# zhaoshan2/pangu-pytorch

Hardware: AMD Instinct MI355X
Metric: forward steps/sec (721x1440x13pl) per MI355X (higher is better)
Workload: dtype f32; 1 GPU; PanguModel fp32 forward, 1 sample/GPU, input (1,5,13,721,1440)+(1,4,721,1440), depths 2-6-6-2, dims 192/384, random-init weights (BASELINE configs[1]); parallelism=dp1

## Files before the change

pangu-pytorch_amd/csrc/gemm_f32_split.hip:

```cpp
#include "split_f32.h"

namespace {

using namespace pangu_split;

using Tile = SplitTile<2, 2, 3>;
constexpr int BM = Tile::BM;
constexpr int BN = Tile::BN;

__global__ __launch_bounds__(256) void split_weight_kernel(const float* __restrict__ W, unsigned char* __restrict__ image, int N,
                                                           int K) {
  const int kc = K >> 3;
  const long long t = (long long)blockIdx.x * 256 + threadIdx.x;
  if (t >= (long long)N * kc) return;
  const int n = (int)(t / kc), c = (int)(t - (long long)n * kc);
  const float* src = W + (size_t)n * K + c * 8;
  const f32x4 c0 = *reinterpret_cast<const f32x4*>(src), c1 = *reinterpret_cast<const f32x4*>(src + 4);
  bf16x8 p[3];
  split8(c0, c1, p[0], p[1], p[2]);
  const int nt = n / BN, nl = n - nt * BN, kt = c >> 1, lh = c & 1;
  unsigned char* dst = image + ((size_t)nt * (K / BK) + kt) * B_BYTES + (lh * BN + nl) * 16;
#pragma unroll
  for (int q = 0; q < 3; ++q) *reinterpret_cast<bf16x8*>(dst + q * PLANE) = p[q];
}

template <int ACT, bool HAS_BIAS>
__global__ __launch_bounds__(256, 2) void gemm_f32_split_kernel(const float* __restrict__ A, int lda,
                                                                const unsigned char* __restrict__ image,
                                                                const float* __restrict__ bias, float* __restrict__ C, int ldc,
                                                                int M, int N, int K, int m_tiles, int n_tiles) {
  __shared__ __attribute__((aligned(16))) unsigned char smem[Tile::SMEM];

  const int b = blockIdx.x;
  const int xcd = b & 7, local = b >> 3;
  const int m_tile = (local / n_tiles) * 8 + xcd;
  const int n_tile = local % n_tiles;
  if (m_tile >= m_tiles) return;
  const int m0 = m_tile * BM, n0 = n_tile * BN;

  const int lane = threadIdx.x & 63;
  const int wave = __builtin_amdgcn_readfirstlane(threadIdx.x >> 6);
  const int wm = wave >> 1, wn = wave & 1;
  const int lr = lane & 31, lh = lane >> 5;

  f32x16 acc[2][3];
  split_main_loop<2, 2, 3>(smem, A, lda, image, M, N, K, m0, n_tile, acc);

  constexpr int EP_LD = 36;
  float* ep = reinterpret_cast<float*>(smem) + wave * (32 * EP_LD);
  const int er = lane >> 3, ec = (lane & 7) * 4;
  const __amdgpu_buffer_rsrc_t c_rsrc = __builtin_amdgcn_make_buffer_rsrc(
      C, 0, (int)(((size_t)(M - 1) * ldc + N) * sizeof(float)), 0x00020000);
#pragma unroll
  for (int j = 0; j < 3; ++j) {
    const int col = n0 + wn * 96 + j * 32 + ec;
    f32x4 bv = {0.f, 0.f, 0.f, 0.f};
    if (HAS_BIAS) bv = *reinterpret_cast<const f32x4*>(bias + col);
#pragma unroll
    for (int i = 0; i < 2; ++i) {
#pragma unroll
      for (int r = 0; r < 16; ++r) ep[((r & 3) + 8 * (r >> 2) + 4 * lh) * EP_LD + lr] = acc[i][j][r];
      const int row0 = m0 + wm * 64 + i * 32 + er;
#pragma unroll
      for (int it = 0; it < 4; ++it) {
        f32x4 v = *reinterpret_cast<const f32x4*>(&ep[(er + 8 * it) * EP_LD + ec]);
        v += bv;
        if (ACT == PANGU_ACT_GELU) {
#pragma unroll
          for (int c = 0; c < 4; ++c) v[c] = gelu_erf(v[c]);
        }
        const unsigned off = ((unsigned)(row0 + 8 * it) * (unsigned)ldc + (unsigned)col) * 4u;
        __builtin_amdgcn_raw_buffer_store_b128(__builtin_bit_cast(u32x4, v), c_rsrc, (int)off, 0, 2);
      }
    }
  }
}

}

extern "C" int pangu_split_weight_bf16x3(pangu_stream_t stream, const float* W, int N, int K, void* image) {
  if (!W || !image) return PANGU_E_NULL;
  if (N <= 0 || K <= 0 || (N % BN) != 0 || (K % BK) != 0) return PANGU_E_SHAPE;
  if ((long long)N * K * 6 >= 0xFFFFFFFFll) return PANGU_E_RANGE;
  const long long threads = (long long)N * (K / 8);
  hipLaunchKernelGGL(split_weight_kernel, dim3((unsigned)((threads + 255) / 256)), dim3(256), 0, (hipStream_t)stream, W,
                     reinterpret_cast<unsigned char*>(image), N, K);
  return pangu_launch_status();
}

extern "C" int pangu_linear_fwd_split(pangu_stream_t stream, const float* A, int lda, const void* image, const float* bias,
                                      float* C, int ldc, int M, int N, int K, int act) {
  if (!A || !image || !C) return PANGU_E_NULL;
  if (M <= 0 || N <= 0 || K <= 0 || lda < K || ldc < N || (lda & 3) || (ldc & 3)) return PANGU_E_SHAPE;
  if (act != PANGU_ACT_NONE && act != PANGU_ACT_GELU) return PANGU_E_ARG;
  if ((N % BN) != 0 || (K % BK) != 0) return PANGU_E_SHAPE;
  if (!pangu_fits_u32(M, lda, 4) || !pangu_fits_u32(M, ldc, 4) || (long long)N * K * 6 >= 0xFFFFFFFFll) return PANGU_E_RANGE;
  const int m_tiles = (M + BM - 1) / BM, n_tiles = N / BN;
  const dim3 g(((m_tiles + 7) / 8) * 8 * n_tiles), blk(256);
  hipStream_t s = (hipStream_t)stream;
  const unsigned char* img = reinterpret_cast<const unsigned char*>(image);
#define PANGU_SPLIT_LAUNCH(ACT, HB) \
  hipLaunchKernelGGL((gemm_f32_split_kernel<ACT, HB>), g, blk, 0, s, A, lda, img, bias, C, ldc, M, N, K, m_tiles, n_tiles)
  if (act == PANGU_ACT_GELU) {
    if (bias) PANGU_SPLIT_LAUNCH(PANGU_ACT_GELU, true); else PANGU_SPLIT_LAUNCH(PANGU_ACT_GELU, false);
  } else {
    if (bias) PANGU_SPLIT_LAUNCH(PANGU_ACT_NONE, true); else PANGU_SPLIT_LAUNCH(PANGU_ACT_NONE, false);
  }
#undef PANGU_SPLIT_LAUNCH
  return pangu_launch_status();
}
```

pangu-pytorch_amd/csrc/gemm_ln_f32_split.hip:

```cpp
#include "ln_epilogue_f32.h"
#include "split_f32.h"

namespace {

using namespace pangu_split;

template <int WMW, int WNW, int NST, bool HAS_BIAS>
__global__ __launch_bounds__(64 * WMW * WNW, WMW * WNW == 8 ? 1 : 2) void gemm_ln_residual_f32_split_kernel(
    const float* __restrict__ A, int lda, const unsigned char* __restrict__ image, const float* __restrict__ bias,
    const float* __restrict__ shortcut, int lds_sc, const float* __restrict__ gamma, const float* __restrict__ beta,
    float* __restrict__ C, int ldc, int M, int K, float branch_scale) {
  using Tile = SplitTile<WMW, WNW, NST>;
  __shared__ __attribute__((aligned(16))) unsigned char smem[Tile::SMEM];
  const int m0 = blockIdx.x * Tile::BM;
  f32x16 acc[2][3];
  split_main_loop<WMW, WNW, NST>(smem, A, lda, image, M, Tile::BN, K, m0, 0, acc);
  pangu_ln::ln_residual_epilogue<WMW, WNW, HAS_BIAS, false>(smem, acc, bias, shortcut, lds_sc, gamma, beta, C, ldc, M, m0,
                                                           branch_scale);
}

template <int WMW, int WNW, int NST>
int launch_ln_split(hipStream_t s, const float* A, int lda, const unsigned char* image, const float* bias, const float* shortcut,
                    int lds, const float* gamma, const float* beta, float* out, int ldo, int M, int K, float branch_scale) {
  constexpr int BM = 64 * WMW;
  dim3 g((M + BM - 1) / BM), blk(64 * WMW * WNW);
  if (bias)
    hipLaunchKernelGGL((gemm_ln_residual_f32_split_kernel<WMW, WNW, NST, true>), g, blk, 0, s, A, lda, image, bias, shortcut, lds,
                       gamma, beta, out, ldo, M, K, branch_scale);
  else
    hipLaunchKernelGGL((gemm_ln_residual_f32_split_kernel<WMW, WNW, NST, false>), g, blk, 0, s, A, lda, image, bias, shortcut, lds,
                       gamma, beta, out, ldo, M, K, branch_scale);
  return pangu_launch_status();
}

}

extern "C" int pangu_linear_ln_residual_fwd_split(pangu_stream_t stream, const float* A, int lda, const void* image,
                                                  const float* bias, const float* shortcut, int lds, const float* gamma,
                                                  const float* beta, float* out, int ldo, int M, int N, int K,
                                                  float branch_scale) {
  if (!A || !image || !shortcut || !gamma || !beta || !out) return PANGU_E_NULL;
  if (M <= 0 || K <= 0 || (K % BK) != 0 || lda < K || (lda & 3) || ldo < N || (ldo & 3) || lds < N || (lds & 3))
    return PANGU_E_SHAPE;
  if (N != 192 && N != 384) return PANGU_E_SHAPE;
  if (!pangu_fits_u32(M, lda, 4) || !pangu_fits_u32(M, ldo, 4) || !pangu_fits_u32(M, lds, 4) ||
      (long long)N * K * 6 >= 0xFFFFFFFFll)
    return PANGU_E_RANGE;
  hipStream_t s = (hipStream_t)stream;
  const unsigned char* img = reinterpret_cast<const unsigned char*>(image);
  if (N == 192) return launch_ln_split<2, 2, 3>(s, A, lda, img, bias, shortcut, lds, gamma, beta, out, ldo, M, K, branch_scale);
  return launch_ln_split<1, 4, 2>(s, A, lda, img, bias, shortcut, lds, gamma, beta, out, ldo, M, K, branch_scale);
}
```

pangu-pytorch_amd/csrc/ln_epilogue_f32.h:

```cpp
#pragma once
#include "common.h"

namespace pangu_ln {

constexpr float LN_EPS = 1e-5f;

__device__ inline float oct_sum(float v) {
  v += __builtin_bit_cast(float, __builtin_amdgcn_update_dpp(0, __builtin_bit_cast(int, v), 0xB1, 0xF, 0xF, true));
  v += __builtin_bit_cast(float, __builtin_amdgcn_update_dpp(0, __builtin_bit_cast(int, v), 0x4E, 0xF, 0xF, true));
  v += __builtin_bit_cast(float, __builtin_amdgcn_update_dpp(0, __builtin_bit_cast(int, v), 0x141, 0xF, 0xF, true));
  return v;
}

template <int WMW, int WNW, bool HAS_BIAS, bool PIN_COL>
__device__ __forceinline__ void ln_residual_epilogue(unsigned char* smem, const f32x16 (&acc)[2][3], const float* __restrict__ bias,
                                                     const float* __restrict__ shortcut, int lds_sc,
                                                     const float* __restrict__ gamma, const float* __restrict__ beta,
                                                     float* __restrict__ C, int ldc, int M, int m0, float branch_scale) {
  constexpr int NW = WMW * WNW;
  constexpr int BN = 96 * WNW;
  constexpr int EP_LD = 36;
  constexpr float INV_C = 1.0f / BN;
  const int lane = threadIdx.x & 63;
  const int wave = __builtin_amdgcn_readfirstlane(threadIdx.x >> 6);
  const int wm = wave / WNW, wn = wave % WNW;
  const int lr = lane & 31, lh = lane >> 5;
  float* ep = reinterpret_cast<float*>(smem) + wave * (32 * EP_LD);
  float* stats = reinterpret_cast<float*>(smem) + NW * (32 * EP_LD);
  const int er = lane >> 3, ec = (lane & 7) * 4;
  const __amdgpu_buffer_rsrc_t c_rsrc = __builtin_amdgcn_make_buffer_rsrc(
      C, 0, (int)(((size_t)(M - 1) * ldc + BN) * sizeof(float)), 0x00020000);
  const __amdgpu_buffer_rsrc_t s_rsrc = __builtin_amdgcn_make_buffer_rsrc(
      const_cast<float*>(shortcut), 0, (int)(((size_t)(M - 1) * lds_sc + BN) * sizeof(float)), 0x00020000);
#pragma unroll
  for (int i = 0; i < 2; ++i) {
    f32x4 y[3][4];
    float s[4] = {0.f, 0.f, 0.f, 0.f}, q[4] = {0.f, 0.f, 0.f, 0.f};
#pragma unroll
    for (int j = 0; j < 3; ++j) {
      int col = wn * 96 + j * 32 + ec;
      if (PIN_COL) asm volatile("" : "+v"(col));
      f32x4 bv = {0.f, 0.f, 0.f, 0.f};
      if (HAS_BIAS) bv = *reinterpret_cast<const f32x4*>(bias + col);
#pragma unroll
      for (int r = 0; r < 16; ++r) ep[((r & 3) + 8 * (r >> 2) + 4 * lh) * EP_LD + lr] = acc[i][j][r];
#pragma unroll
      for (int it = 0; it < 4; ++it) {
        f32x4 v = *reinterpret_cast<const f32x4*>(&ep[(er + 8 * it) * EP_LD + ec]);
        v += bv;
        y[j][it] = v;
        s[it] += (v[0] + v[1]) + (v[2] + v[3]);
        q[it] += (v[0] * v[0] + v[1] * v[1]) + (v[2] * v[2] + v[3] * v[3]);
      }
    }
#pragma unroll
    for (int it = 0; it < 4; ++it) {
      const float ss = oct_sum(s[it]), qq = oct_sum(q[it]);
      if ((lane & 7) == 0) {
        float* st = stats + (((wm * WNW + wn) * 64) + i * 32 + er + 8 * it) * 2;
        st[0] = ss;
        st[1] = qq;
      }
    }
    __syncthreads();
    float mean[4], rstd[4];
#pragma unroll
    for (int it = 0; it < 4; ++it) {
      const int rloc = i * 32 + er + 8 * it;
      float ts = 0.f, tq = 0.f;
#pragma unroll
      for (int w = 0; w < WNW; ++w) {
        const float* st = stats + ((wm * WNW + w) * 64 + rloc) * 2;
        ts += st[0];
        tq += st[1];
      }
      mean[it] = ts * INV_C;
      rstd[it] = rsqrtf(fmaxf(tq * INV_C - mean[it] * mean[it], 0.f) + LN_EPS);
    }
#pragma unroll
    for (int j = 0; j < 3; ++j) {
      int col = wn * 96 + j * 32 + ec;
      if (PIN_COL) asm volatile("" : "+v"(col));
      const f32x4 gm = *reinterpret_cast<const f32x4*>(gamma + col);
      const f32x4 bt = *reinterpret_cast<const f32x4*>(beta + col);
#pragma unroll
      for (int it = 0; it < 4; ++it) {
        const unsigned row = (unsigned)(m0 + wm * 64 + i * 32 + er + 8 * it);
        const f32x4 sc = __builtin_bit_cast(
            f32x4, __builtin_amdgcn_raw_buffer_load_b128(s_rsrc, (int)((row * (unsigned)lds_sc + (unsigned)col) * 4u), 0, 0));
        const f32x4 v = sc + branch_scale * ((y[j][it] - mean[it]) * rstd[it] * gm + bt);
        __builtin_amdgcn_raw_buffer_store_b128(__builtin_bit_cast(u32x4, v), c_rsrc,
                                               (int)((row * (unsigned)ldc + (unsigned)col) * 4u), 0, 0);
      }
    }
  }
}

}
```

pangu-pytorch_amd/csrc/split_f32.h:

```cpp
#pragma once
#include "gemm_f32_dma_loop.h"

namespace pangu_split {

using pangu_dma::BK;
using pangu_dma::kswz64;

typedef short bf16x8 __attribute__((ext_vector_type(8)));

constexpr int W_ROWS = 192;
constexpr int PLANE = 2 * W_ROWS * 16;
constexpr int B_BYTES = 3 * PLANE;
constexpr int W_PIECES = B_BYTES / 1024;

__device__ inline void split2(float a, float b, unsigned& hi, unsigned& mid, unsigned& lo) {
  const bf16x2_t h = __builtin_convertvector(f32x2_t{a, b}, bf16x2_t);
  const f32x2_t r1 = f32x2_t{a, b} - __builtin_convertvector(h, f32x2_t);
  const bf16x2_t m = __builtin_convertvector(r1, bf16x2_t);
  const f32x2_t r2 = r1 - __builtin_convertvector(m, f32x2_t);
  hi = __builtin_bit_cast(unsigned, h);
  mid = __builtin_bit_cast(unsigned, m);
  lo = __builtin_bit_cast(unsigned, __builtin_convertvector(r2, bf16x2_t));
}

__device__ inline void split8(const f32x4 c0, const f32x4 c1, bf16x8& hi, bf16x8& mid, bf16x8& lo) {
  unsigned h0, h1, h2, h3, m0, m1, m2, m3, l0, l1, l2, l3;
  split2(c0[0], c0[1], h0, m0, l0);
  split2(c0[2], c0[3], h1, m1, l1);
  split2(c1[0], c1[1], h2, m2, l2);
  split2(c1[2], c1[3], h3, m3, l3);
  hi = __builtin_bit_cast(bf16x8, u32x4{h0, h1, h2, h3});
  mid = __builtin_bit_cast(bf16x8, u32x4{m0, m1, m2, m3});
  lo = __builtin_bit_cast(bf16x8, u32x4{l0, l1, l2, l3});
}

template <int WMW, int WNW, int NST>
struct SplitTile {
  static constexpr int NW = WMW * WNW;
  static constexpr int BM = 64 * WMW;
  static constexpr int BN = 96 * WNW;
  static constexpr int NT = BN / W_ROWS;
  static constexpr int A_BYTES = BM * 64;
  static constexpr int STAGE = A_BYTES + NT * B_BYTES;
  static constexpr int SMEM = NST * STAGE;
  static_assert(NST == 2 || NST == 3, "ring depth");
  static_assert(BN % W_ROWS == 0, "whole n-tile blocks");
};

template <int WMW, int WNW, int NST>
__device__ __forceinline__ void split_main_loop(unsigned char* smem, const float* __restrict__ A, int lda,
                                                const unsigned char* __restrict__ image, int M, int N, int K, int m0,
                                                int first_n_tile, f32x16 (&acc)[2][3]) {
  using T = SplitTile<WMW, WNW, NST>;
  constexpr int NW = T::NW, A_BYTES = T::A_BYTES, STAGE = T::STAGE;
  constexpr int A_PIECES = A_BYTES / 1024;
  constexpr int PIECES = STAGE / 1024;
  constexpr int A_IT = A_PIECES / NW;
  constexpr int IT = (PIECES + NW - 1) / NW;
  constexpr int REM = PIECES % NW;
  static_assert(A_PIECES % NW == 0, "piece rounds");

  const int tid = threadIdx.x, lane = tid & 63;
  const int wave = __builtin_amdgcn_readfirstlane(tid >> 6);
  const int wm = wave / WNW, wn = wave % WNW;
  const int lr = lane & 31, lh = lane >> 5;
  const int KT = K / BK;

  const __amdgpu_buffer_rsrc_t a_rsrc = __builtin_amdgcn_make_buffer_rsrc(
      const_cast<float*>(A), 0, (int)(((size_t)(M - 1) * lda + K) * sizeof(float)), 0x00020000);
  const __amdgpu_buffer_rsrc_t w_rsrc = __builtin_amdgcn_make_buffer_rsrc(
      const_cast<unsigned char*>(image), 0, (int)((size_t)N * K * 6), 0x00020000);
  unsigned voff_a[A_IT], voff_w[IT - A_IT];
#pragma unroll
  for (int i = 0; i < A_IT; ++i) {
    const int row = 16 * (i * NW + wave) + (lane >> 2);
    const int f = (0x78 >> (((row >> 2) & 3) * 2)) & 3;
    voff_a[i] = ((unsigned)(m0 + row) * (unsigned)lda + ((lane & 3) ^ f) * 4) * 4u;
  }
#pragma unroll
  for (int i = A_IT; i < IT; ++i) {
    const int p = i * NW + wave - A_PIECES;
    voff_w[i - A_IT] = (unsigned)(first_n_tile + p / W_PIECES) * (unsigned)KT * (unsigned)B_BYTES +
                       (unsigned)(p % W_PIECES) * 1024u + lane * 16;
  }
  auto issue = [&](int kt, int slot) {
    unsigned char* base = smem + slot * STAGE;
#pragma unroll
    for (int i = 0; i < IT; ++i) {
      const int q = i * NW + wave;
      auto dst = (__attribute__((address_space(3))) void*)(base + q * 1024);
      if (i < A_IT) {
        __builtin_amdgcn_raw_ptr_buffer_load_lds(a_rsrc, dst, 16, (int)voff_a[i], kt * BK * 4, 0, 0);
      } else if (i * NW + NW - 1 < PIECES || q < PIECES) {
        __builtin_amdgcn_raw_ptr_buffer_load_lds(w_rsrc, dst, 16, (int)voff_w[i - A_IT], kt * B_BYTES, 0, 0);
      }
    }
  };

#pragma unroll
  for (int i = 0; i < 2; ++i)
#pragma unroll
    for (int j = 0; j < 3; ++j)
#pragma unroll
      for (int r = 0; r < 16; ++r) acc[i][j][r] = 0.f;

  int off_a[2][2];
#pragma unroll
  for (int i = 0; i < 2; ++i)
#pragma unroll
    for (int h = 0; h < 2; ++h) off_a[i][h] = kswz64(wm * 64 + i * 32 + lr, 2 * lh + h);
  const int off_w = A_BYTES + (wn >> 1) * B_BYTES + (lh * W_ROWS + (wn & 1) * 96 + lr) * 16;

  issue(0, 0);
  if (NST == 3 && KT > 1) issue(1, 1);
  int slot = 0;
  for (int kt = 0; kt < KT; ++kt) {
    if (NST == 3 && kt + 1 < KT) {
      if (REM == 0 || wave < REM) asm volatile("s_waitcnt vmcnt(%0)" ::"n"(IT) : "memory");
      else asm volatile("s_waitcnt vmcnt(%0)" ::"n"(IT - 1) : "memory");
    } else {
      asm volatile("s_waitcnt vmcnt(0)" ::: "memory");
    }
    __builtin_amdgcn_s_barrier();
    asm volatile("" ::: "memory");
    if (NST == 3) {
      if (kt + 2 < KT) issue(kt + 2, slot == 0 ? 2 : slot - 1);
    } else {
      if (kt + 1 < KT) issue(kt + 1, slot ^ 1);
    }
    const unsigned char* St = smem + slot * STAGE;
    slot = slot == NST - 1 ? 0 : slot + 1;

    bf16x8 bw[3][3];
#pragma unroll
    for (int j = 0; j < 3; ++j)
#pragma unroll
      for (int p = 0; p < 3; ++p) bw[j][p] = *reinterpret_cast<const bf16x8*>(St + off_w + p * PLANE + j * 512);
    f32x4 ca[2][2];
#pragma unroll
    for (int i = 0; i < 2; ++i)
#pragma unroll
      for (int h = 0; h < 2; ++h) ca[i][h] = *reinterpret_cast<const f32x4*>(St + off_a[i][h]);
    bf16x8 ah[2], am[2], al[2];
    split8(ca[0][0], ca[0][1], ah[0], am[0], al[0]);
    auto products = [&](int i) {
#pragma unroll
      for (int j = 0; j < 3; ++j) {
        acc[i][j] = __builtin_amdgcn_mfma_f32_32x32x16_bf16(al[i], bw[j][0], acc[i][j], 0, 0, 0);
        acc[i][j] = __builtin_amdgcn_mfma_f32_32x32x16_bf16(ah[i], bw[j][2], acc[i][j], 0, 0, 0);
        acc[i][j] = __builtin_amdgcn_mfma_f32_32x32x16_bf16(am[i], bw[j][1], acc[i][j], 0, 0, 0);
        acc[i][j] = __builtin_amdgcn_mfma_f32_32x32x16_bf16(am[i], bw[j][0], acc[i][j], 0, 0, 0);
        acc[i][j] = __builtin_amdgcn_mfma_f32_32x32x16_bf16(ah[i], bw[j][1], acc[i][j], 0, 0, 0);
        acc[i][j] = __builtin_amdgcn_mfma_f32_32x32x16_bf16(ah[i], bw[j][0], acc[i][j], 0, 0, 0);
      }
    };
    __builtin_amdgcn_sched_barrier(0);
    products(0);
    split8(ca[1][0], ca[1][1], ah[1], am[1], al[1]);
#pragma unroll
    for (int g = 0; g < 18; ++g) {
      __builtin_amdgcn_sched_group_barrier(0x008, 1, 0);
      __builtin_amdgcn_sched_group_barrier(0x002, 3, 0);
    }
    __builtin_amdgcn_sched_barrier(0);
    products(1);
  }
  __syncthreads();
}

}
```

pangu-pytorch_amd/split_layout.py:

```python

BM, BN, BK = 128, 192, 16
A_BYTES = BM * 64
PLANE = 2 * BN * 16
B_BYTES = 3 * PLANE
STAGE = A_BYTES + B_BYTES
PLANES = ("hi", "mid", "lo")
_F = (0, 2, 3, 1)


def served(N, K):
    return N % BN == 0 and K % BK == 0


def image_index(N, K, plane, n, k):
    nt, nl, kt, lh, j = n // BN, n % BN, k // BK, (k // 8) & 1, k % 8
    return (((((nt * (K // BK) + kt) * 3 + plane) * 2 + lh) * BN + nl) * 8) + j


def unpermute(image_u16, N, K):
    return [[[image_u16[image_index(N, K, p, n, k)] for k in range(K)] for n in range(N)] for p in range(3)]


def a_chunk_offset(row, chunk):
    return row * 64 + ((chunk ^ _F[(row >> 2) & 3]) << 4)


def a_fragment_address(lane, wm, i, h):
    return a_chunk_offset(wm * 64 + i * 32 + (lane & 31), 2 * (lane >> 5) + h)


def w_fragment_address(lane, wn, j, plane):
    return A_BYTES + plane * PLANE + ((lane >> 5) * BN + wn * 96 + j * 32 + (lane & 31)) * 16


def dma_piece_destination(q, lane):
    return q * 1024 + lane * 16
```

Baseline: 19.96 forward steps/s.

## Add row-owning warp tiling for split-bf16x3 GEMMs with lean register schedule

Adds a ROWS variant of the split-bf16x3 tile, where each wave owns 32 rows by six 32-column blocks instead of 64x96. The plain GEMM switches to a 4x1 wave layout with two pipeline stages, three blocks per CU, and a lean schedule that streams weight fragments between MFMA groups to lower register pressure. The GEMM+LayerNorm path gains a row-owning epilogue used for wide N when K>=1536. This trades A-fragment reuse and a pipeline stage for more occupancy and fewer registers, and it reworks scheduling hints.

```diff
diff --git a/pangu-pytorch_amd/csrc/gemm_f32_split.hip b/pangu-pytorch_amd/csrc/gemm_f32_split.hip
--- a/pangu-pytorch_amd/csrc/gemm_f32_split.hip
+++ b/pangu-pytorch_amd/csrc/gemm_f32_split.hip
@@ -4,7 +4,7 @@
 
 using namespace pangu_split;
 
-using Tile = SplitTile<2, 2, 3>;
+using Tile = SplitTile<4, 1, 2, true>;
 constexpr int BM = Tile::BM;
 constexpr int BN = Tile::BN;
 
@@ -25,7 +25,7 @@
 }
 
 template <int ACT, bool HAS_BIAS>
-__global__ __launch_bounds__(256, 2) void gemm_f32_split_kernel(const float* __restrict__ A, int lda,
+__global__ __launch_bounds__(256, 3) void gemm_f32_split_kernel(const float* __restrict__ A, int lda,
                                                                 const unsigned char* __restrict__ image,
                                                                 const float* __restrict__ bias, float* __restrict__ C, int ldc,
                                                                 int M, int N, int K, int m_tiles, int n_tiles) {
@@ -40,38 +40,34 @@
 
   const int lane = threadIdx.x & 63;
   const int wave = __builtin_amdgcn_readfirstlane(threadIdx.x >> 6);
-  const int wm = wave >> 1, wn = wave & 1;
   const int lr = lane & 31, lh = lane >> 5;
 
-  f32x16 acc[2][3];
-  split_main_loop<2, 2, 3>(smem, A, lda, image, M, N, K, m0, n_tile, acc);
+  f32x16 acc[1][6];
+  split_main_loop<4, 1, 2, true, true>(smem, A, lda, image, M, N, K, m0, n_tile, acc);
 
   constexpr int EP_LD = 36;
   float* ep = reinterpret_cast<float*>(smem) + wave * (32 * EP_LD);
   const int er = lane >> 3, ec = (lane & 7) * 4;
   const __amdgpu_buffer_rsrc_t c_rsrc = __builtin_amdgcn_make_buffer_rsrc(
       C, 0, (int)(((size_t)(M - 1) * ldc + N) * sizeof(float)), 0x00020000);
+  const int row0 = m0 + wave * 32 + er;
 #pragma unroll
-  for (int j = 0; j < 3; ++j) {
-    const int col = n0 + wn * 96 + j * 32 + ec;
+  for (int j = 0; j < 6; ++j) {
+    const int col = n0 + j * 32 + ec;
     f32x4 bv = {0.f, 0.f, 0.f, 0.f};
     if (HAS_BIAS) bv = *reinterpret_cast<const f32x4*>(bias + col);
 #pragma unroll
-    for (int i = 0; i < 2; ++i) {
+    for (int r = 0; r < 16; ++r) ep[((r & 3) + 8 * (r >> 2) + 4 * lh) * EP_LD + lr] = acc[0][j][r];
 #pragma unroll
-      for (int r = 0; r < 16; ++r) ep[((r & 3) + 8 * (r >> 2) + 4 * lh) * EP_LD + lr] = acc[i][j][r];
-      const int row0 = m0 + wm * 64 + i * 32 + er;
+    for (int it = 0; it < 4; ++it) {
+      f32x4 v = *reinterpret_cast<const f32x4*>(&ep[(er + 8 * it) * EP_LD + ec]);
+      v += bv;
+      if (ACT == PANGU_ACT_GELU) {
 #pragma unroll
-      for (int it = 0; it < 4; ++it) {
-        f32x4 v = *reinterpret_cast<const f32x4*>(&ep[(er + 8 * it) * EP_LD + ec]);
-        v += bv;
-        if (ACT == PANGU_ACT_GELU) {
-#pragma unroll
-          for (int c = 0; c < 4; ++c) v[c] = gelu_erf(v[c]);
-        }
-        const unsigned off = ((unsigned)(row0 + 8 * it) * (unsigned)ldc + (unsigned)col) * 4u;
-        __builtin_amdgcn_raw_buffer_store_b128(__builtin_bit_cast(u32x4, v), c_rsrc, (int)off, 0, 2);
+        for (int c = 0; c < 4; ++c) v[c] = gelu_erf(v[c]);
       }
+      const unsigned off = ((unsigned)(row0 + 8 * it) * (unsigned)ldc + (unsigned)col) * 4u;
+      __builtin_amdgcn_raw_buffer_store_b128(__builtin_bit_cast(u32x4, v), c_rsrc, (int)off, 0, 2);
     }
   }
 }
diff --git a/pangu-pytorch_amd/csrc/gemm_ln_f32_split.hip b/pangu-pytorch_amd/csrc/gemm_ln_f32_split.hip
--- a/pangu-pytorch_amd/csrc/gemm_ln_f32_split.hip
+++ b/pangu-pytorch_amd/csrc/gemm_ln_f32_split.hip
@@ -5,31 +5,35 @@
 
 using namespace pangu_split;
 
-template <int WMW, int WNW, int NST, bool HAS_BIAS>
+template <int WMW, int WNW, int NST, bool ROWS, bool HAS_BIAS>
 __global__ __launch_bounds__(64 * WMW * WNW, WMW * WNW == 8 ? 1 : 2) void gemm_ln_residual_f32_split_kernel(
     const float* __restrict__ A, int lda, const unsigned char* __restrict__ image, const float* __restrict__ bias,
     const float* __restrict__ shortcut, int lds_sc, const float* __restrict__ gamma, const float* __restrict__ beta,
     float* __restrict__ C, int ldc, int M, int K, float branch_scale) {
-  using Tile = SplitTile<WMW, WNW, NST>;
+  using Tile = SplitTile<WMW, WNW, NST, ROWS>;
   __shared__ __attribute__((aligned(16))) unsigned char smem[Tile::SMEM];
   const int m0 = blockIdx.x * Tile::BM;
-  f32x16 acc[2][3];
-  split_main_loop<WMW, WNW, NST>(smem, A, lda, image, M, Tile::BN, K, m0, 0, acc);
-  pangu_ln::ln_residual_epilogue<WMW, WNW, HAS_BIAS, false>(smem, acc, bias, shortcut, lds_sc, gamma, beta, C, ldc, M, m0,
-                                                           branch_scale);
+  f32x16 acc[Tile::RB][Tile::CB];
+  split_main_loop<WMW, WNW, NST, ROWS>(smem, A, lda, image, M, Tile::BN, K, m0, 0, acc);
+  if constexpr (ROWS)
+    pangu_ln::ln_residual_epilogue_rows<WMW, WNW, HAS_BIAS>(smem, acc, bias, shortcut, lds_sc, gamma, beta, C, ldc, M, m0,
+                                                            branch_scale);
+  else
+    pangu_ln::ln_residual_epilogue<WMW, WNW, HAS_BIAS, false>(smem, acc, bias, shortcut, lds_sc, gamma, beta, C, ldc, M, m0,
+                                                             branch_scale);
 }
 
-template <int WMW, int WNW, int NST>
+template <int WMW, int WNW, int NST, bool ROWS>
 int launch_ln_split(hipStream_t s, const float* A, int lda, const unsigned char* image, const float* bias, const float* shortcut,
                     int lds, const float* gamma, const float* beta, float* out, int ldo, int M, int K, float branch_scale) {
-  constexpr int BM = 64 * WMW;
+  constexpr int BM = SplitTile<WMW, WNW, NST, ROWS>::BM;
   dim3 g((M + BM - 1) / BM), blk(64 * WMW * WNW);
   if (bias)
-    hipLaunchKernelGGL((gemm_ln_residual_f32_split_kernel<WMW, WNW, NST, true>), g, blk, 0, s, A, lda, image, bias, shortcut, lds,
-                       gamma, beta, out, ldo, M, K, branch_scale);
+    hipLaunchKernelGGL((gemm_ln_residual_f32_split_kernel<WMW, WNW, NST, ROWS, true>), g, blk, 0, s, A, lda, image, bias, shortcut,
+                       lds, gamma, beta, out, ldo, M, K, branch_scale);
   else
-    hipLaunchKernelGGL((gemm_ln_residual_f32_split_kernel<WMW, WNW, NST, false>), g, blk, 0, s, A, lda, image, bias, shortcut, lds,
-                       gamma, beta, out, ldo, M, K, branch_scale);
+    hipLaunchKernelGGL((gemm_ln_residual_f32_split_kernel<WMW, WNW, NST, ROWS, false>), g, blk, 0, s, A, lda, image, bias, shortcut,
+                       lds, gamma, beta, out, ldo, M, K, branch_scale);
   return pangu_launch_status();
 }
 
@@ -48,6 +52,7 @@
     return PANGU_E_RANGE;
   hipStream_t s = (hipStream_t)stream;
   const unsigned char* img = reinterpret_cast<const unsigned char*>(image);
-  if (N == 192) return launch_ln_split<2, 2, 3>(s, A, lda, img, bias, shortcut, lds, gamma, beta, out, ldo, M, K, branch_scale);
-  return launch_ln_split<1, 4, 2>(s, A, lda, img, bias, shortcut, lds, gamma, beta, out, ldo, M, K, branch_scale);
+  if (N == 192) return launch_ln_split<2, 2, 3, false>(s, A, lda, img, bias, shortcut, lds, gamma, beta, out, ldo, M, K, branch_scale);
+  if (K < 1536) return launch_ln_split<1, 4, 2, false>(s, A, lda, img, bias, shortcut, lds, gamma, beta, out, ldo, M, K, branch_scale);
+  return launch_ln_split<2, 2, 2, true>(s, A, lda, img, bias, shortcut, lds, gamma, beta, out, ldo, M, K, branch_scale);
 }
diff --git a/pangu-pytorch_amd/csrc/ln_epilogue_f32.h b/pangu-pytorch_amd/csrc/ln_epilogue_f32.h
--- a/pangu-pytorch_amd/csrc/ln_epilogue_f32.h
+++ b/pangu-pytorch_amd/csrc/ln_epilogue_f32.h
@@ -96,4 +96,88 @@
   }
 }
 
+template <int WMW, int WNW, bool HAS_BIAS>
+__device__ __forceinline__ void ln_residual_epilogue_rows(unsigned char* smem, const f32x16 (&acc)[1][6],
+                                                          const float* __restrict__ bias, const float* __restrict__ shortcut,
+                                                          int lds_sc, const float* __restrict__ gamma,
+                                                          const float* __restrict__ beta, float* __restrict__ C, int ldc, int M,
+                                                          int m0, float branch_scale) {
+  constexpr int NW = WMW * WNW;
+  constexpr int BN = 192 * WNW;
+  constexpr int NG = 2 * WNW;
+  constexpr int EP_LD = 36;
+  constexpr float INV_C = 1.0f / BN;
+  const int lane = threadIdx.x & 63;
+  const int wave = __builtin_amdgcn_readfirstlane(threadIdx.x >> 6);
+  const int wm = wave / WNW, wn = wave % WNW;
+  const int lr = lane & 31, lh = lane >> 5;
+  float* ep = reinterpret_cast<float*>(smem) + wave * (32 * EP_LD);
+  float* stats = reinterpret_cast<float*>(smem) + NW * (32 * EP_LD);
+  const int er = lane >> 3, ec = (lane & 7) * 4;
+  const __amdgpu_buffer_rsrc_t c_rsrc = __builtin_amdgcn_make_buffer_rsrc(
+      C, 0, (int)(((size_t)(M - 1) * ldc + BN) * sizeof(float)), 0x00020000);
+  const __amdgpu_buffer_rsrc_t s_rsrc = __builtin_amdgcn_make_buffer_rsrc(
+      const_cast<float*>(shortcut), 0, (int)(((size_t)(M - 1) * lds_sc + BN) * sizeof(float)), 0x00020000);
+  f32x4 y[6][4];
+#pragma unroll
+  for (int g = 0; g < 2; ++g) {
+    float s[4] = {0.f, 0.f, 0.f, 0.f}, q[4] = {0.f, 0.f, 0.f, 0.f};
+#pragma unroll
+    for (int jj = 0; jj < 3; ++jj) {
+      const int j = 3 * g + jj;
+      const int col = wn * 192 + j * 32 + ec;
+      f32x4 bv = {0.f, 0.f, 0.f, 0.f};
+      if (HAS_BIAS) bv = *reinterpret_cast<const f32x4*>(bias + col);
+#pragma unroll
+      for (int r = 0; r < 16; ++r) ep[((r & 3) + 8 * (r >> 2) + 4 * lh) * EP_LD + lr] = acc[0][j][r];
+#pragma unroll
+      for (int it = 0; it < 4; ++it) {
+        f32x4 v = *reinterpret_cast<const f32x4*>(&ep[(er + 8 * it) * EP_LD + ec]);
+        v += bv;
+        y[j][it] = v;
+        s[it] += (v[0] + v[1]) + (v[2] + v[3]);
+        q[it] += (v[0] * v[0] + v[1] * v[1]) + (v[2] * v[2] + v[3] * v[3]);
+      }
+    }
+#pragma unroll
+    for (int it = 0; it < 4; ++it) {
+      const float ss = oct_sum(s[it]), qq = oct_sum(q[it]);
+      if ((lane & 7) == 0) {
+        float* st = stats + ((wm * NG + 2 * wn + g) * 32 + er + 8 * it) * 2;
+        st[0] = ss;
+        st[1] = qq;
+      }
+    }
+  }
+  __syncthreads();
+  float mean[4], rstd[4];
+#pragma unroll
+  for (int it = 0; it < 4; ++it) {
+    float ts = 0.f, tq = 0.f;
+#pragma unroll
+    for (int g = 0; g < NG; ++g) {
+      const float* st = stats + ((wm * NG + g) * 32 + er + 8 * it) * 2;
+      ts += st[0];
+      tq += st[1];
+    }
+    mean[it] = ts * INV_C;
+    rstd[it] = rsqrtf(fmaxf(tq * INV_C - mean[it] * mean[it], 0.f) + LN_EPS);
+  }
+#pragma unroll
+  for (int j = 0; j < 6; ++j) {
+    const int col = wn * 192 + j * 32 + ec;
+    const f32x4 gm = *reinterpret_cast<const f32x4*>(gamma + col);
+    const f32x4 bt = *reinterpret_cast<const f32x4*>(beta + col);
+#pragma unroll
+    for (int it = 0; it < 4; ++it) {
+      const unsigned row = (unsigned)(m0 + wm * 32 + er + 8 * it);
+      const f32x4 sc = __builtin_bit_cast(
+          f32x4, __builtin_amdgcn_raw_buffer_load_b128(s_rsrc, (int)((row * (unsigned)lds_sc + (unsigned)col) * 4u), 0, 0));
+      const f32x4 v = sc + branch_scale * ((y[j][it] - mean[it]) * rstd[it] * gm + bt);
+      __builtin_amdgcn_raw_buffer_store_b128(__builtin_bit_cast(u32x4, v), c_rsrc,
+                                             (int)((row * (unsigned)ldc + (unsigned)col) * 4u), 0, 0);
+    }
+  }
 }
+
+}
diff --git a/pangu-pytorch_amd/csrc/split_f32.h b/pangu-pytorch_amd/csrc/split_f32.h
--- a/pangu-pytorch_amd/csrc/split_f32.h
+++ b/pangu-pytorch_amd/csrc/split_f32.h
@@ -34,11 +34,13 @@
   lo = __builtin_bit_cast(bf16x8, u32x4{l0, l1, l2, l3});
 }
 
-template <int WMW, int WNW, int NST>
+template <int WMW, int WNW, int NST, bool ROWS>
 struct SplitTile {
+  static constexpr int RB = ROWS ? 1 : 2;
+  static constexpr int CB = ROWS ? 6 : 3;
   static constexpr int NW = WMW * WNW;
-  static constexpr int BM = 64 * WMW;
-  static constexpr int BN = 96 * WNW;
+  static constexpr int BM = 32 * RB * WMW;
+  static constexpr int BN = 32 * CB * WNW;
   static constexpr int NT = BN / W_ROWS;
   static constexpr int A_BYTES = BM * 64;
   static constexpr int STAGE = A_BYTES + NT * B_BYTES;
@@ -47,12 +49,13 @@
   static_assert(BN % W_ROWS == 0, "whole n-tile blocks");
 };
 
-template <int WMW, int WNW, int NST>
+template <int WMW, int WNW, int NST, bool ROWS, bool LEAN = false>
 __device__ __forceinline__ void split_main_loop(unsigned char* smem, const float* __restrict__ A, int lda,
                                                 const unsigned char* __restrict__ image, int M, int N, int K, int m0,
-                                                int first_n_tile, f32x16 (&acc)[2][3]) {
-  using T = SplitTile<WMW, WNW, NST>;
-  constexpr int NW = T::NW, A_BYTES = T::A_BYTES, STAGE = T::STAGE;
+                                                int first_n_tile,
+                                                f32x16 (&acc)[SplitTile<WMW, WNW, NST, ROWS>::RB][SplitTile<WMW, WNW, NST, ROWS>::CB]) {
+  using T = SplitTile<WMW, WNW, NST, ROWS>;
+  constexpr int NW = T::NW, A_BYTES = T::A_BYTES, STAGE = T::STAGE, RB = T::RB, CB = T::CB;
   constexpr int A_PIECES = A_BYTES / 1024;
   constexpr int PIECES = STAGE / 1024;
   constexpr int A_IT = A_PIECES / NW;
@@ -98,18 +101,19 @@
   };
 
 #pragma unroll
-  for (int i = 0; i < 2; ++i)
-#pragma unroll
-    for (int j = 0; j < 3; ++j)
+  for (int i = 0; i < RB; ++i)
+#pragma unroll
+    for (int j = 0; j < CB; ++j)
 #pragma unroll
       for (int r = 0; r < 16; ++r) acc[i][j][r] = 0.f;
 
-  int off_a[2][2];
-#pragma unroll
-  for (int i = 0; i < 2; ++i)
-#pragma unroll
-    for (int h = 0; h < 2; ++h) off_a[i][h] = kswz64(wm * 64 + i * 32 + lr, 2 * lh + h);
-  const int off_w = A_BYTES + (wn >> 1) * B_BYTES + (lh * W_ROWS + (wn & 1) * 96 + lr) * 16;
+  int off_a[RB][2];
+#pragma unroll
+  for (int i = 0; i < RB; ++i)
+#pragma unroll
+    for (int h = 0; h < 2; ++h) off_a[i][h] = kswz64((wm * RB + i) * 32 + lr, 2 * lh + h);
+  const int wcol = wn * CB * 32;
+  const int off_w = A_BYTES + (wcol / W_ROWS) * B_BYTES + (lh * W_ROWS + wcol % W_ROWS + lr) * 16;
 
   issue(0, 0);
   if (NST == 3 && KT > 1) issue(1, 1);
@@ -131,39 +135,66 @@
     const unsigned char* St = smem + slot * STAGE;
     slot = slot == NST - 1 ? 0 : slot + 1;
 
-    bf16x8 bw[3][3];
-#pragma unroll
-    for (int j = 0; j < 3; ++j)
-#pragma unroll
-      for (int p = 0; p < 3; ++p) bw[j][p] = *reinterpret_cast<const bf16x8*>(St + off_w + p * PLANE + j * 512);
-    f32x4 ca[2][2];
-#pragma unroll
-    for (int i = 0; i < 2; ++i)
+    bf16x8 bw[CB][3];
+    f32x4 ca[RB][2];
+    auto read_w = [&](int j0, int j1) {
+#pragma unroll
+      for (int j = j0; j < j1; ++j)
+#pragma unroll
+        for (int p = 0; p < 3; ++p) bw[j][p] = *reinterpret_cast<const bf16x8*>(St + off_w + p * PLANE + j * 512);
+    };
+    read_w(0, LEAN ? 3 : CB);
+#pragma unroll
+    for (int i = 0; i < RB; ++i)
 #pragma unroll
       for (int h = 0; h < 2; ++h) ca[i][h] = *reinterpret_cast<const f32x4*>(St + off_a[i][h]);
-    bf16x8 ah[2], am[2], al[2];
-    split8(ca[0][0], ca[0][1], ah[0], am[0], al[0]);
+    bf16x8 ah[RB], am[RB], al[RB];
+    auto tile = [&](int i, int j) {
+      acc[i][j] = __builtin_amdgcn_mfma_f32_32x32x16_bf16(al[i], bw[j][0], acc[i][j], 0, 0, 0);
+      acc[i][j] = __builtin_amdgcn_mfma_f32_32x32x16_bf16(ah[i], bw[j][2], acc[i][j], 0, 0, 0);
+      acc[i][j] = __builtin_amdgcn_mfma_f32_32x32x16_bf16(am[i], bw[j][1], acc[i][j], 0, 0, 0);
+      acc[i][j] = __builtin_amdgcn_mfma_f32_32x32x16_bf16(am[i], bw[j][0], acc[i][j], 0, 0, 0);
+      acc[i][j] = __builtin_amdgcn_mfma_f32_32x32x16_bf16(ah[i], bw[j][1], acc[i][j], 0, 0, 0);
+      acc[i][j] = __builtin_amdgcn_mfma_f32_32x32x16_bf16(ah[i], bw[j][0], acc[i][j], 0, 0, 0);
+    };
     auto products = [&](int i) {
 #pragma unroll
-      for (int j = 0; j < 3; ++j) {
-        acc[i][j] = __builtin_amdgcn_mfma_f32_32x32x16_bf16(al[i], bw[j][0], acc[i][j], 0, 0, 0);
-        acc[i][j] = __builtin_amdgcn_mfma_f32_32x32x16_bf16(ah[i], bw[j][2], acc[i][j], 0, 0, 0);
-        acc[i][j] = __builtin_amdgcn_mfma_f32_32x32x16_bf16(am[i], bw[j][1], acc[i][j], 0, 0, 0);
-        acc[i][j] = __builtin_amdgcn_mfma_f32_32x32x16_bf16(am[i], bw[j][0], acc[i][j], 0, 0, 0);
-        acc[i][j] = __builtin_amdgcn_mfma_f32_32x32x16_bf16(ah[i], bw[j][1], acc[i][j], 0, 0, 0);
-        acc[i][j] = __builtin_amdgcn_mfma_f32_32x32x16_bf16(ah[i], bw[j][0], acc[i][j], 0, 0, 0);
+      for (int j = 0; j < CB; ++j) tile(i, j);
+    };
+    if constexpr (ROWS) {
+      if constexpr (LEAN) {
+        static_assert(CB == 6, "three tiles ahead");
+        __builtin_amdgcn_sched_barrier(0);
+        split8(ca[0][0], ca[0][1], ah[0], am[0], al[0]);
+        __builtin_amdgcn_sched_barrier(0);
+#pragma unroll
+        for (int j = 0; j < 3; ++j) {
+          tile(0, j);
+          read_w(j + 3, j + 4);
+          __builtin_amdgcn_sched_barrier(0);
+        }
+#pragma unroll
+        for (int j = 3; j < CB; ++j) tile(0, j);
+      } else {
+        split8(ca[0][0], ca[0][1], ah[0], am[0], al[0]);
+        __builtin_amdgcn_sched_group_barrier(0x100, 2 + 3 * CB, 0);
+        __builtin_amdgcn_sched_group_barrier(0x002, 40, 0);
+        products(0);
       }
-    };
-    __builtin_amdgcn_sched_barrier(0);
-    products(0);
-    split8(ca[1][0], ca[1][1], ah[1], am[1], al[1]);
-#pragma unroll
-    for (int g = 0; g < 18; ++g) {
-      __builtin_amdgcn_sched_group_barrier(0x008, 1, 0);
-      __builtin_amdgcn_sched_group_barrier(0x002, 3, 0);
-    }
-    __builtin_amdgcn_sched_barrier(0);
-    products(1);
+    } else {
+      static_assert(!LEAN, "LEAN is a schedule of the row-owning tiling");
+      split8(ca[0][0], ca[0][1], ah[0], am[0], al[0]);
+      __builtin_amdgcn_sched_barrier(0);
+      products(0);
+      split8(ca[1][0], ca[1][1], ah[1], am[1], al[1]);
+#pragma unroll
+      for (int g = 0; g < 18; ++g) {
+        __builtin_amdgcn_sched_group_barrier(0x008, 1, 0);
+        __builtin_amdgcn_sched_group_barrier(0x002, 3, 0);
+      }
+      __builtin_amdgcn_sched_barrier(0);
+      products(1);
+    }
   }
   __syncthreads();
 }
diff --git a/pangu-pytorch_amd/split_layout.py b/pangu-pytorch_amd/split_layout.py
--- a/pangu-pytorch_amd/split_layout.py
+++ b/pangu-pytorch_amd/split_layout.py
@@ -33,5 +33,13 @@
     return A_BYTES + plane * PLANE + ((lane >> 5) * BN + wn * 96 + j * 32 + (lane & 31)) * 16
 
 
+def a_row_fragment_address(lane, wm, h):
+    return a_chunk_offset(wm * 32 + (lane & 31), 2 * (lane >> 5) + h)
+
+
+def w_row_fragment_address(lane, wn, j, plane, a_bytes=A_BYTES):
+    return a_bytes + wn * B_BYTES + plane * PLANE + ((lane >> 5) * BN + j * 32 + (lane & 31)) * 16
+
+
 def dma_piece_destination(q, lane):
     return q * 1024 + lane * 16
```

After: 20.46 forward steps/s (median of 6 runs). 1.03x the previous value.
